# olga24912/lodestar

Hardware: AMD Instinct MI355X
Metric: verified signature sets/sec (node) (higher is better)
Workload: dtype u32/u64 (28-bit-limb Montgomery integer arithmetic); 1 GPU; C2 gossip attestation flood: 16384 single-pubkey sets per GPU, 1 set per batchable job; pk_mode=device table, sig_encoding=compressed 96 B, distinct_messages=16384, group_sets=1024, group_policy=0, inflight=32, slots=3, hw_queues=4, merge_sets=131072, pipeline_depth=3, parallelism=shard-by-job x1 (in-process devices), no collective

## Files before the change

lodestar_amd/csrc/helpers.cpp:

```cpp
#include "helper_layout.hpp"
#include "runtime_internal.hpp"

using namespace blsgpu_rt;
namespace hl = helper_layout;

static_assert(hl::kFp == W_FP && hl::kG1A == W_G1A && hl::kG1J == W_G1J && hl::kG2A == W_G2A && hl::kG2J == W_G2J &&
                  hl::kFp12 == W_FP12 && hl::kAwrTabWords == AWR_TAB_WORDS && hl::kMillerLineWords == kMillerLineWords,
              "helper_layout.hpp restates the element widths of kernels.h");

namespace {

template <class Body>
int helper_call(blsgpu_ctx* ctx, bool reads_table, Body body) {
  if (!enter(ctx)) return BLSGPU_ERR_CLOSED;
  struct Leave {
    blsgpu_ctx* ctx;
    ~Leave() { leave(ctx); }
  } leave_on_exit{ctx};
  Device& d = *ctx->devs[0];
  try {
    std::lock_guard<std::mutex> helper(d.helper_mu);
    std::shared_lock<std::shared_mutex> tl(d.table_mu, std::defer_lock);
    if (reads_table) tl.lock();
    HIPCHK(hipSetDevice(d.id));
// ... 447 lines not shown
    return BLSGPU_OK;
  });
}

int blsgpu_signing_roots(blsgpu_ctx* ctx, int kind, uint32_t n, const uint8_t* objects, uint32_t object_stride,
                         const uint8_t* domains, uint32_t domain_stride, uint8_t* out32) {
  if (!ctx || ctx->devs.empty() || !objects || !domains || !out32) return BLSGPU_ERR_ARGS;
  const uint32_t obj_len = kind == BLSGPU_ROOT_OBJECT ? 32 : (kind == BLSGPU_ROOT_ATTESTATION_DATA ? 128 : 0);
  if (!obj_len || object_stride < obj_len || (domain_stride != 0 && domain_stride < 32)) return BLSGPU_ERR_ARGS;
  if (n == 0) return BLSGPU_OK;
  return helper_call(ctx, false, [&](Device& d, Slot& sl, hipStream_t s) -> int {
    const hl::SigningRoots l(n, object_stride, domain_stride);
    sl.d_in.ensure(l.total);
    uint8_t* din = sl.d_in.p;
    HIPCHK(hipMemcpyAsync(din, objects, (size_t)n * object_stride, hipMemcpyHostToDevice, s));
    HIPCHK(hipMemcpyAsync(din + l.dom, domains, l.dom_bytes, hipMemcpyHostToDevice, s));
    launch_signing_roots(kind, din, n, object_stride, din + l.dom, domain_stride, din + l.out, s);
    HIPCHK(hipGetLastError());
    HIPCHK(hipMemcpyAsync(out32, din + l.out, 32 * (size_t)n, hipMemcpyDeviceToHost, s));
    HIPCHK(hipStreamSynchronize(s));
    return BLSGPU_OK;
  });
}

int blsgpu_debug_op(blsgpu_ctx* ctx, int op, uint32_t n, const uint8_t* in, uint32_t in_stride, uint8_t* out,
                    uint32_t out_stride, int32_t* status) {
  if (!ctx || ctx->devs.empty() || !in || !out || !status) return BLSGPU_ERR_ARGS;
  struct OpSize {
    int op;
    uint32_t in, out;
  };
  static const OpSize kOpSizes[] = {{0, 96, 48},    {1, 194, 192},  {2, 32, 192},   {3, 288, 576},  {4, 576, 576},
                                    {5, 104, 96},   {6, 200, 192},  {7, 64, 96},    {8, 32, 96},    {9, 200, 2880},
                                    {10, 104, 1440}, {11, 840, 56}, {16, 576, 576}, {17, 288, 576}, {18, 384, 192}};
  const OpSize* sz = nullptr;
  for (const OpSize& o : kOpSizes)
    if (o.op == op) sz = &o;
  if (!sz || in_stride < sz->in || out_stride < sz->out) return BLSGPU_ERR_ARGS;
  if (n == 0) return BLSGPU_OK;
  return helper_call(ctx, false, [&](Device& d, Slot& sl, hipStream_t s) -> int {
    struct Temp {
      void* p = nullptr;
      ~Temp() {
        if (p) (void)hipFree(p);
      }
    } din, dout, dst;
    HIPCHK(hipMalloc(&din.p, (size_t)n * in_stride));
    HIPCHK(hipMalloc(&dout.p, (size_t)n * out_stride));
    HIPCHK(hipMalloc(&dst.p, (size_t)n * 4));
    HIPCHK(hipMemcpyAsync(din.p, in, (size_t)n * in_stride, hipMemcpyHostToDevice, s));
    HIPCHK(hipMemsetAsync(dout.p, 0, (size_t)n * out_stride, s));
    launch_debug_op(op, n, (uint8_t*)din.p, in_stride, (uint8_t*)dout.p, out_stride, (int32_t*)dst.p, s);
    HIPCHK(hipGetLastError());
    HIPCHK(hipMemcpyAsync(out, dout.p, (size_t)n * out_stride, hipMemcpyDeviceToHost, s));
    HIPCHK(hipMemcpyAsync(status, dst.p, (size_t)n * 4, hipMemcpyDeviceToHost, s));
    HIPCHK(hipStreamSynchronize(s));
    return BLSGPU_OK;
  });
}

}
```

lodestar_amd/csrc/k_common.hpp:

```cpp
#pragma once
#include <atomic>

#include "kernels.h"
#include "ops.hpp"
#include "fp2x.hpp"

#define WAVE 64
#if defined(__HIP_DEVICE_COMPILE__) && !BLS_INLINE_PRODUCTS && !BLS_FP2_CLASSIC
static_assert(WAVE <= BLS_FP2_LDS_LANES, "fp2_mul LDS slot");
static_assert(2 * WAVE <= BLS_FP2_LDS_LANES, "128-lane kernels (gt_wave.hpp, k_msm_bucket) and fp2_mul LDS slot");
#endif

#ifndef BLSGPU_WPE
#define BLSGPU_WPE 1
#endif
#define STAGE_KERNEL __global__ __launch_bounds__(WAVE) __attribute__((amdgpu_waves_per_eu(BLSGPU_WPE, BLSGPU_WPE)))
#define STAGE_KERNEL_W(w) __global__ __launch_bounds__(WAVE) __attribute__((amdgpu_waves_per_eu(w, w)))
#ifndef BLSGPU_WPE_PK
#define BLSGPU_WPE_PK BLSGPU_WPE
#endif
#ifndef BLSGPU_WPE_HPREP
#define BLSGPU_WPE_HPREP 1
#endif
#ifndef BLSGPU_WPE_MSM
#define BLSGPU_WPE_MSM BLSGPU_WPE
#endif
#ifndef BLSGPU_WPE_LINES
#define BLSGPU_WPE_LINES BLSGPU_WPE
#endif
#ifndef BLSGPU_WPE_ACC
#define BLSGPU_WPE_ACC BLSGPU_WPE
#endif
#ifndef BLSGPU_WPE_DEC
#define BLSGPU_WPE_DEC BLSGPU_WPE
#endif
#ifndef BLSGPU_WPE_HASH
#define BLSGPU_WPE_HASH BLSGPU_WPE
#endif
#ifndef BLSGPU_WPE_HMAP
#define BLSGPU_WPE_HMAP 2
#endif
#ifndef BLSGPU_WPE_GRP
#define BLSGPU_WPE_GRP BLSGPU_WPE
#endif

__device__ __forceinline__ uint32_t opaque_u32(uint32_t x) {
  asm volatile("" : "+v"(x));
  return x;
}

__device__ __forceinline__ fp ld_fp(const uint32_t* p, uint32_t n, uint32_t i, int w0) {
  fp r;
// ... 154 lines not shown
  }
  return r;
}

template <class F>
__device__ jac<F> jac_mul_u64_j(const jac<F>& P, uint64_t k) {
  jac<F> r = jac_infinity<F>();
  if (k == 0) return r;
  int top = 63;
  while (((k >> top) & 1ull) == 0) top--;
  r = P;
  for (int i = top - 1; i >= 0; i--) {
    r = jac_dbl(r);
    if ((k >> i) & 1ull) r = jac_add(r, P);
  }
  return r;
}

template <class F>
__device__ __forceinline__ void tab_st(uint32_t* tab, uint32_t n, uint32_t i, int e, const jac<F>& v) {
  constexpr int WF = sizeof(F) / 4;
  const uint32_t* s = reinterpret_cast<const uint32_t*>(&v);
#pragma unroll
  for (int w = 0; w < 3 * WF; w++) tab[((size_t)e * 3 * WF + w) * n + i] = s[w];
}
template <class F>
__device__ __forceinline__ jac<F> tab_ld(const uint32_t* tab, uint32_t n, uint32_t i, int e) {
  constexpr int WF = sizeof(F) / 4;
  jac<F> v;
  uint32_t* d = reinterpret_cast<uint32_t*>(&v);
#pragma unroll
  for (int w = 0; w < 3 * WF; w++) d[w] = tab[((size_t)e * 3 * WF + w) * n + i];
  return v;
}
BLS_HD int scalar_word_digit(uint64_t w, int k, bool& neg) {
  const int d = 2 * (int)((w >> (4 * k)) & 15u) - 15;
  neg = d < 0;
  return (d < 0 ? -d : d) >> 1;
}
template <class F>
__device__ jac<F> jac_mul_scalar_word(const jac<F>& P, uint64_t w, uint32_t* tab, uint32_t n, uint32_t i) {
  const jac<F> P2 = jac_dbl(P);
  jac<F> t = P;
  tab_st(tab, n, i, 0, t);
#pragma unroll 1
  for (int e = 1; e < 8; e++) {
    t = jac_add(t, P2);
    tab_st(tab, n, i, e, t);
  }
  const uint32_t ii = opaque_u32(i);
  auto term = [&](int k, bool hi) {
    bool neg;
    const int e = scalar_word_digit(w, hi ? k + 8 : k, neg);
    jac<F> q = tab_ld<F>(tab, n, ii, e);
    if (hi) q = endo_lambda(q);
    return neg ? jac_neg(q) : q;
  };
  jac<F> r = jac_add(term(7, false), term(7, true));
#pragma unroll 1
  for (int k = 6; k >= 0; k--) {
    r = jac_dbl(jac_dbl(jac_dbl(jac_dbl(r))));
    r = jac_add(r, term(k, false));
    r = jac_add(r, term(k, true));
  }
  return r;
}

template <class F>
__device__ jac<F> jac_mul_words(const jac<F>& P, const uint32_t* k, int nw) {
  jac<F> r = jac_infinity<F>();
  for (int i = 32 * nw - 1; i >= 0; i--) {
// ... 34 lines not shown
```

lodestar_amd/csrc/k_debug.hip:

```cpp
#include "k_common.hpp"
#include "gt_wave.hpp"

__device__ fp dbg_load_fp(const uint8_t* b) {
  fp x;
  fp_from_be48_plain(b, x, 0xff);
  return fp_to_mont(x);
}
__device__ fp2 dbg_load_fp2(const uint8_t* b) { return fp2_make(dbg_load_fp(b + 48), dbg_load_fp(b)); }
__device__ g2a dbg_load_g2(const uint8_t* b) {
  g2a p;
  p.x = dbg_load_fp2(b);
  p.y = dbg_load_fp2(b + 96);
  return p;
}
__device__ g1a dbg_load_g1(const uint8_t* b) {
  g1a p;
  p.x = dbg_load_fp(b);
  p.y = dbg_load_fp(b + 48);
  return p;
}
__device__ void dbg_store_fp12(const fp12& f, uint8_t* b) {
  const fp2* c[6] = {&f.c0.c0, &f.c0.c1, &f.c0.c2, &f.c1.c0, &f.c1.c1, &f.c1.c2};
  for (int k = 0; k < 6; k++) {
    fp_to_be48(c[k]->c0, b + 96 * k);
// ... 82 lines not shown
      g1a pk;
      st = jac_to_aff(jac_mul_words(jac_from_aff(g), w, 8), pk) ? 0 : -1;
      if (st == 0) g1a_to_be96(pk, o);
      break;
    }
    case 9: {
      uint64_t w = 0;
      for (int j = 0; j < 8; j++) w |= (uint64_t)a[192 + j] << (8 * j);
      g2a r;
      uint32_t* tab = reinterpret_cast<uint32_t*>(o + 192);
      st = jac_to_aff(jac_mul_scalar_word(jac_from_aff(dbg_load_g2(a)), w, tab, 1, 0), r) ? 0 : -1;
      if (st == 0) g2a_to_be192(r, o);
      break;
    }
    case 10: {
      uint64_t w = 0;
      for (int j = 0; j < 8; j++) w |= (uint64_t)a[96 + j] << (8 * j);
      g1a r;
      uint32_t* tab = reinterpret_cast<uint32_t*>(o + 96);
      st = jac_to_aff(jac_mul_scalar_word(jac_from_aff(dbg_load_g1(a)), w, tab, 1, 0), r) ? 0 : -1;
      if (st == 0) g1a_to_be96(r, o);
      break;
    }
    case 11: {
      const uint32_t* w = reinterpret_cast<const uint32_t*>(a);
      fp x[15];
      for (int k = 0; k < 15; k++)
        for (int j = 0; j < BLS_NL; j++) x[k].l[j] = w[14 * k + j];
      const fp r = fp_lc(T<1>(x[0]), T<1>(x[1]), T<1>(x[2]), T<1>(x[3]), T<1>(x[4]), T<1>(x[5]), T<1>(x[6]),
                         T<-1>(x[7]), T<-1>(x[8]), T<-1>(x[9]), T<-1>(x[10]), T<-1>(x[11]), T<-1>(x[12]), T<-1>(x[13]),
                         T<-1>(x[14]));
      uint32_t* ow = reinterpret_cast<uint32_t*>(o);
      for (int j = 0; j < BLS_NL; j++) ow[j] = r.l[j];
      break;
    }
    default:
      st = -2;
  }
  status[i] = st;
}

__global__ __launch_bounds__(GTW_MILLER_LANES) void k_debug_gt(int op, const uint8_t* in, uint32_t in_stride, uint8_t* out,
                                                         uint32_t out_stride, int32_t* status) {
  __shared__ GtwLds sh;
  const uint32_t i = blockIdx.x, t = threadIdx.x;
  const uint8_t* a = in + (size_t)i * in_stride;
  uint8_t* o = out + (size_t)i * out_stride;
  if (op == 16) {
    if (t == 0) gtw_from_reg(sh.F, dbg_load_fp12(a));
    gtw_sync();
    gtw_final_exp(sh.F, sh.W, sh.S, t);
  } else {
    if (t == 0) {
      const g1a P = dbg_load_g1(a);
      const g2a Q = dbg_load_g2(a + 96);
      lds_st(sh.QA, 0, Q.x.c0);
      lds_st(sh.QA, 1, Q.x.c1);
      lds_st(sh.QA, 2, Q.y.c0);
      lds_st(sh.QA, 3, Q.y.c1);
      lds_st(sh.L, 0, P.x);
      lds_st(sh.L, 1, P.y);
    }
    gtw_sync();
    const fp xP = lds_ld(sh.L, 0), yP = lds_ld(sh.L, 1);
    gtw_sync();
    gtw_miller_loop(sh.F, sh.QA, xP, yP, sh.TB, sh.L, sh.L1, sh.S, sh.S2, t);
// ... 87 lines not shown
```

lodestar_amd/csrc/k_pk.hip:

```cpp
#include "k_common.hpp"

#ifndef BLSGPU_PK_AGG_GROUPS
#define BLSGPU_PK_AGG_GROUPS 1
#endif
__global__ __launch_bounds__(WAVE) void k_pk_aggregate(PipelineBuffers b, uint32_t n_sets) {
  __shared__ uint32_t red[WAVE * W_G1J];
  __shared__ uint32_t err_k[WAVE];
  __shared__ int32_t err_c[WAVE];
  if (blockIdx.x >= n_sets) return;
  const uint32_t set = b.agg_sets ? b.agg_sets[blockIdx.x] : blockIdx.x;
  uint32_t lane = threadIdx.x;
  int8_t* agg_status = b.status + 2 * b.n;
  const uint32_t first = b.set_pk_first[set], last = b.set_pk_first[set + 1];
  g1j acc = jac_infinity<fp>();
  uint32_t my_err_k = 0xffffffffu;
  int my_err = 0;
  for (uint32_t k = first + lane; k < last; k += WAVE) {
    g1a q;
    if (b.pk_bytes) {
      uint8_t raw[96];
      const uint8_t* src = b.pk_bytes + (size_t)k * 96;
#pragma unroll
      for (int t = 0; t < 96; t++) raw[t] = src[t];
      bool inf = false;
// ... 146 lines not shown
      uint4 v = src[k];
      uint32_t w[4] = {v.x, v.y, v.z, v.w};
#pragma unroll
      for (int j = 0; j < 16; j++) raw[16 * k + j] = (uint8_t)(w[j >> 2] >> (8 * (j & 3)));
    }
    g1a a;
    bool inf = false;
    int st = pk_decode96(raw, a, inf);
    if (st == BLS_OK && inf) st = BLS_PK_IS_INFINITY;
    if (st == BLS_OK) P = jac_from_aff(a);
    return st;
  }
  if (b.set_pk_first[i + 1] == b.set_pk_first[i]) return BLS_EMPTY_AGGREGATE;
  const int st = b.status[2 * b.n + i];
  if (st) return st;
  P = ld_g1j(b.pk_jac, b.n, i);
  return jac_is_inf(P) ? BLS_PK_IS_INFINITY : BLS_OK;
}

STAGE_KERNEL_W(BLSGPU_WPE_PK) void k_pk_finish(PipelineBuffers b, uint32_t n_sets, int8_t* pk_status) {
  uint32_t i = blockIdx.x * WAVE + threadIdx.x;
  if (i >= n_sets) return;
  g1j P;
  int st = set_pubkey(b, i, P);
  g1j R = jac_infinity<fp>();
  if (st == BLS_OK) {
    const uint64_t w = b.scalars[i];
    R = (w == 0) ? P : jac_mul_scalar_word(P, w, b.scal_tab, b.n, i);
  }
  st_g1j(b.pk_jac, b.n, i, R);
  pk_status[i] = (int8_t)st;
}

STAGE_KERNEL void k_unit_aggregate(PipelineBuffers b) {
  uint32_t u = blockIdx.x * WAVE + threadIdx.x;
  if (u >= b.n_units) return;
  const uint32_t a = b.unit_set_first[u], e = b.unit_set_first[u + 1];
  g1a out;
  out.x = fp_zero();
  out.y = fp_zero();
  bool ok = false;
  if (e - a == 1) {
    const uint32_t i = b.unit_sets[a];
    if (b.include[i]) {
      out = ld_g1a(b.pk_aff, b.n, i);
      ok = true;
    }
  } else {
    g1j acc = jac_infinity<fp>();
    for (uint32_t k = a; k < e; k++) {
      const uint32_t i = b.unit_sets[k];
      if (b.include[i]) acc = jac_add_aff(acc, ld_g1a(b.pk_aff, b.n, i));
    }
    ok = jac_to_aff(acc, out);
  }
  st_g1a(b.unit_p, b.n, u, out);
  b.unit_ok[u] = ok ? 1 : 0;
}

__global__ __launch_bounds__(WAVE) void k_pk_serialize(PipelineBuffers b, uint32_t n_sets, uint8_t* out,
                                                       uint32_t out_len) {
  uint32_t i = blockIdx.x * WAVE + threadIdx.x;
  if (i >= n_sets) return;
  int st = b.set_pk_first[i + 1] == b.set_pk_first[i] ? BLS_EMPTY_AGGREGATE : b.status[2 * b.n + i];
  uint8_t buf[96];
  for (int k = 0; k < 96; k++) buf[k] = 0;
// ... 21 lines not shown
  for (uint32_t k = 0; k < 96; k++) raw[k] = k < pk_len ? src[k] : 0;
  g1a a;
  const int st = pk_key_validate(raw, pk_len, a);
  uint8_t buf[96];
  for (int k = 0; k < 96; k++) buf[k] = 0;
  if (st == BLS_OK) g1a_to_be96(a, buf);
  if (out96)
    for (int k = 0; k < 96; k++) out96[(size_t)i * 96 + k] = buf[k];
  status[i] = (int8_t)st;
}

__global__ __launch_bounds__(WAVE) void k_pk_table_fill(const uint8_t* pk96, uint32_t n, uint32_t* table_dst,
                                                        int8_t* status) {
  uint32_t i = blockIdx.x * WAVE + threadIdx.x;
  if (i >= n) return;
  uint8_t raw[96];
  for (int k = 0; k < 96; k++) raw[k] = pk96[(size_t)i * 96 + k];
  g1a a;
  bool inf = false;
  int st = pk_decode96(raw, a, inf);
  if (st == BLS_OK && inf) st = BLS_PK_IS_INFINITY;
  uint32_t* dst = table_dst + (size_t)i * W_PKTAB;
  for (int l = 0; l < BLS_NL; l++) {
    dst[l] = st == BLS_OK ? a.x.l[l] : 0;
    dst[BLS_NL + l] = st == BLS_OK ? a.y.l[l] : 0;
  }
  dst[2 * BLS_NL] = 0;
  dst[2 * BLS_NL + 1] = 0;
  dst[2 * BLS_NL + 2] = 0;
  dst[2 * BLS_NL + 3] = 0;
  status[i] = (int8_t)st;
}

static inline dim3 grid_for(uint32_t n) { return dim3((n + WAVE - 1) / WAVE); }

void launch_pk_aggregate(const PipelineBuffers& b, uint32_t n, hipStream_t s) {
  if (b.agg_sets) n = b.n_agg;
  if (!n) return;
  const uint32_t lanes = 1024 * WAVE;
  if ((uint64_t)n * 64 <= lanes || !BLSGPU_PK_AGG_GROUPS)
    hipLaunchKernelGGL(k_pk_aggregate, dim3(n), dim3(WAVE), 0, s, b, n);
  else if ((uint64_t)n * 32 <= 2 * lanes)
    hipLaunchKernelGGL(k_pk_aggregate_g<32>, dim3((n * 32 + WAVE - 1) / WAVE), dim3(WAVE), 0, s, b, n);
  else if ((uint64_t)n * 16 <= 2 * lanes)
    hipLaunchKernelGGL(k_pk_aggregate_g<16>, dim3((n * 16 + WAVE - 1) / WAVE), dim3(WAVE), 0, s, b, n);
  else
    hipLaunchKernelGGL(k_pk_aggregate_g<8>, dim3((n * 8 + WAVE - 1) / WAVE), dim3(WAVE), 0, s, b, n);
}
void launch_pk_finish(const PipelineBuffers& b, uint32_t n, hipStream_t s) {
  if (n) hipLaunchKernelGGL(k_pk_finish, grid_for(n), dim3(WAVE), 0, s, b, n, b.status + b.n);
}
void launch_unit_aggregate(const PipelineBuffers& b, hipStream_t s) {
  if (b.n_units) hipLaunchKernelGGL(k_unit_aggregate, grid_for(b.n_units), dim3(WAVE), 0, s, b);
}
void launch_pk_serialize(const PipelineBuffers& b, uint32_t n, uint8_t* out, uint32_t out_len, hipStream_t s) {
  if (n) hipLaunchKernelGGL(k_pk_serialize, grid_for(n), dim3(WAVE), 0, s, b, n, out, out_len);
}
void launch_key_validate(const uint8_t* pks, uint32_t n, uint32_t pk_len, uint32_t stride, uint8_t* out96,
                         int8_t* status, hipStream_t s) {
  if (n) hipLaunchKernelGGL(k_key_validate, grid_for(n), dim3(WAVE), 0, s, pks, n, pk_len, stride, out96, status);
}
void launch_pk_table_fill(const uint8_t* pk96, uint32_t n, uint32_t* table_dst, int8_t* status, hipStream_t s) {
  if (n) hipLaunchKernelGGL(k_pk_table_fill, grid_for(n), dim3(WAVE), 0, s, pk96, n, table_dst, status);
}
```

lodestar_amd/csrc/kernels.h:

```cpp
#pragma once
#include <hip/hip_runtime.h>
#include <stdint.h>
#include <vector>

#define W_FP 14
#define W_G1A (2 * W_FP)
#define W_G1J (3 * W_FP)
#define W_G2A (4 * W_FP)
#define W_G2J (6 * W_FP)
#define W_FP12 (12 * W_FP)
#define W_PKTAB 32
#define MILLER_STEPS 68
#define W_LINE (3 * 2 * W_FP)

#define SF_SIG_INF 1u
#define MF_H_INF 1u

struct PipelineBuffers {
  uint32_t n;
  const uint8_t* sigs;
  const uint32_t* sig_len;
  uint32_t sig_stride;
  const uint8_t* pk_bytes;
  const uint32_t* set_pk_first;
  const uint32_t* pk_index;
  const uint32_t* pk_table;
  uint32_t pk_table_n;
  const uint32_t* agg_sets;
  uint32_t n_agg;
  uint32_t pk_direct1;
  const uint64_t* scalars;
  uint32_t* scal_tab;
  const uint32_t* job_first_set;
  uint32_t n_jobs;
  const uint8_t* umsgs;
  const uint32_t* msg_idx;
  uint32_t n_umsg;
  uint32_t nm;
  uint32_t n_units;
  const uint32_t* unit_set_first;
  const uint32_t* unit_sets;
  const uint32_t* unit_msg;
  uint32_t* sig_aff;
  uint32_t* h_aff;
  uint32_t* h_jac;
  uint32_t* h_norm;
  uint32_t* h_prep;
  uint32_t* h_q;
  uint32_t* inv_buf;
  uint32_t* inv_buf_pk;
  uint32_t* pk_jac;
  uint32_t* pk_aff;
  uint32_t* rsig;
  uint32_t* unit_p;
  uint32_t n_chunks;
  const uint32_t* chunk_first;
  const uint32_t* chunk_items;
  uint32_t* f_chunk;
  uint32_t* lines;
  uint8_t* flags;
// ... 37 lines not shown
  uint32_t dbl[MILLER_MAX_SEGS];
};
void launch_miller_acc(const PipelineBuffers& b, bool units, hipStream_t s, const MillerSegs* segs = nullptr);
void launch_miller_acc2(const PipelineBuffers& b, bool units, hipStream_t s);
void launch_miller_acc6(const PipelineBuffers& b, bool units, hipStream_t s);
#ifndef BLSGPU_EXCLUSIVE_SMALL
#define BLSGPU_EXCLUSIVE_SMALL 1
#endif
void launch_miller_coop(const PipelineBuffers& b, bool units, hipStream_t s, bool exclusive = false);
void launch_group_reduce(const PipelineBuffers& b, const uint32_t* f_ranges, uint32_t n_groups, uint32_t* F,
                         hipStream_t s);
void launch_group_tree(const PipelineBuffers& b, const uint32_t* f_ranges, uint32_t n_groups, const uint32_t* runs,
                       uint32_t n_runs, const uint32_t* pairs, const std::vector<uint32_t>& level_end, uint32_t* F,
                       hipStream_t s, const MillerSegs* segs = nullptr, uint32_t* H = nullptr);
void launch_group_check(const uint32_t* S, const uint32_t* F, uint32_t n_groups, uint8_t* ok, hipStream_t s,
                        const uint32_t* sel = nullptr, uint32_t n_sel = 0, const uint32_t* G = nullptr,
                        bool exclusive = false, bool lane = false);
void launch_group_check6(const uint32_t* F, const uint32_t* G, uint32_t n_groups, uint8_t* ok, hipStream_t s,
                         const uint32_t* sel = nullptr, uint32_t n_sel = 0);
void launch_check6_miller(const uint32_t* S, const uint32_t* F, uint32_t n_groups, uint8_t* ok, hipStream_t s,
                          const uint32_t* sel, uint32_t n_sel, uint32_t* lines, uint8_t* flags);
void launch_group_sig_miller_sel(const uint32_t* S, uint32_t n_groups, const uint32_t* sel, uint32_t n_sel, uint32_t* G,
                                 hipStream_t s);
void launch_group_sig_miller(const uint32_t* S, uint32_t n_groups, uint32_t* G, hipStream_t s, bool exclusive = false,
                             bool lane = false);
void launch_copy_words(uint32_t* dst, const uint32_t* src, size_t n, hipStream_t s);
void launch_group_reduce_lane(const PipelineBuffers& b, const uint32_t* set_ranges, const uint32_t* f_ranges,
                              uint32_t n_groups, uint32_t* S, uint32_t* F, hipStream_t s);
void launch_range_combine_lane(const uint32_t* S_in, const uint32_t* F_in, uint32_t n_in, const uint32_t* ranges,
                               uint32_t n_out, uint32_t* S_out, uint32_t* F_out, hipStream_t s);
void launch_range_combine(const uint32_t* S_in, const uint32_t* F_in, uint32_t n_in, const uint32_t* ranges,
                          uint32_t n_out, uint32_t* S_out, uint32_t* F_out, hipStream_t s);
void launch_pk_table_fill(const uint8_t* pk96, uint32_t n, uint32_t* table_dst, int8_t* status, hipStream_t s);
void launch_pk_serialize(const PipelineBuffers& b, uint32_t n_sets, uint8_t* out, uint32_t out_len, hipStream_t s);
void launch_key_validate(const uint8_t* pks, uint32_t n, uint32_t pk_len, uint32_t stride, uint8_t* out96,
                         int8_t* status, hipStream_t s);
inline uint32_t sig_agg_lanes(uint32_t n_groups, uint32_t n_sigs) {
  if (n_groups == 0) return 1;
  const uint64_t n = n_groups, lanes = 1024 * 64;
  const uint32_t by_count = n * 64 <= lanes ? 64 : n * 32 <= 2 * lanes ? 32 : n * 16 <= 2 * lanes ? 16
                            : n * 8 <= 2 * lanes ? 8 : 1;
  const uint64_t mean = ((uint64_t)n_sigs + n - 1) / n;
  const uint32_t by_size = mean <= 3 ? 1 : mean <= 8 ? 8 : mean <= 16 ? 16 : mean <= 32 ? 32 : 64;
  return by_count < by_size ? by_count : by_size;
}
void launch_sig_aggregate(const PipelineBuffers& b, const uint32_t* group_first, uint32_t n_groups, uint32_t n_sigs,
                          uint32_t* agg, int8_t* agg_status, uint32_t* first_bad, hipStream_t s);
void launch_sig_agg_serialize(const uint32_t* group_first, uint32_t n_groups, const uint32_t* agg, int8_t* agg_status,
                              uint8_t* out, uint32_t out_len, hipStream_t s);
struct AwrBuffers {
  uint32_t n;
  uint32_t n_groups;
  const uint32_t* group_first;
  const uint64_t* words;
  const uint8_t* pk_bytes;
  const uint32_t* pk_index;
  const uint32_t* pk_table;
  uint32_t pk_table_n;
  const uint32_t* sig_aff;
  const uint8_t* sig_flags;
  const int8_t* sig_status;
  uint32_t* tab;
  uint32_t tab_n;
  uint32_t* sum_pk;
  uint32_t* sum_sig;
  uint32_t* err_k;
// ... 31 lines not shown
```

lodestar_amd/csrc/runtime.cpp:

```cpp
#include <pthread.h>
#include <stdio.h>
#include <sys/random.h>

#include <cmath>
#include <string>
#include <system_error>

#include "runtime_internal.hpp"
#include "miller_plan.hpp"

using namespace blsgpu_rt;

namespace {

std::atomic<int64_t> g_fail_run_skip{0}, g_fail_run_count{0};
thread_local bool tl_dispatcher = false;

inline uint32_t chunk_size(uint32_t len, uint32_t min_per_chunk) {
  const uint32_t count = min_per_chunk ? len / min_per_chunk : 0;
  return count <= 1 ? len : (len + count - 1) / count;
}

struct GroupPlanEntry {
  uint32_t first, end;
// ... 461 lines not shown
  const size_t ob_flags = 0, ob_mflags = al256(n), ob_unit = al256(ob_mflags + nm), ob_status = al256(ob_unit + n),
               ob_include = al256(ob_status + 3 * (size_t)stride), ob_spec = al256(ob_include + stride),
               bytes_total = al256(ob_spec + stride);
  sl.d_bytes.ensure(bytes_total);
  const uint32_t max_ranges = std::max<uint32_t>(std::max(ng0, nj), 1);
  const size_t o_ok = al256(nj), res_bytes = o_ok + max_ranges;
  sl.d_res.ensure(res_bytes);
  sl.h_res.ensure(res_bytes);
  sl.d_S.ensure((size_t)W_G2J * max_ranges);
  sl.d_F.ensure((size_t)W_FP12 * max_ranges);
  sl.d_G.ensure((size_t)W_FP12 * std::max<uint32_t>(ng0, 1));
  sl.d_msmB.ensure((size_t)MSM_BUCKET_WORDS * std::max<uint32_t>(n_slices, 1));
  sl.d_msmW.ensure((size_t)MSM_WINDOW_WORDS * max_ranges);
  const size_t per_set = W_G2A + W_G1J + W_G1A + W_FP12 + 8 * W_G1J + 2 * W_FP + (merged ? W_G1A : 0);
  sl.d_work.ensure((size_t)stride * per_set + (size_t)nm * (W_G2A + W_G2J + W_FP + 14 * W_FP + 2 * W_G2J));
  sl.d_lines.ensure((size_t)nm * kMillerLineWords);
  if (keep_f) sl.d_fkeep.ensure((size_t)stride * W_FP12);
  if (segs > 1) sl.d_fseg.ensure((size_t)W_FP12 * n_franges);
  if (rsig_spec) sl.d_fb.ensure((size_t)stride * 9 * W_G2J);
  uint8_t* const din = sl.d_in.p;
  uint8_t* const d_ok0 = sl.d_res.p + o_ok;

  PipelineBuffers pb;
  memset(&pb, 0, sizeof pb);
  pb.n = stride;
  pb.sigs = din + o_sigs;
  pb.sig_len = reinterpret_cast<uint32_t*>(din + o_siglen);
  pb.sig_stride = sig_w;
  pb.pk_bytes = table_mode ? nullptr : din + (bytes_agg ? o_pk2 : o_pk);
  pb.set_pk_first = (table_mode || bytes_agg) ? reinterpret_cast<uint32_t*>(din + o_pk) : nullptr;
  pb.pk_index = table_mode ? reinterpret_cast<uint32_t*>(din + o_pk2) : nullptr;
  pb.pk_table = d.table.p;
  pb.pk_table_n = d.table_n;
  pb.agg_sets = reinterpret_cast<uint32_t*>(din + o_agg);
  pb.n_agg = (uint32_t)agg_sets.size();
  pb.pk_direct1 = 1;
  pb.scalars = reinterpret_cast<uint64_t*>(din + o_scal);
  pb.job_first_set = reinterpret_cast<uint32_t*>(din + o_jobs);
  pb.n_jobs = nj;
  pb.umsgs = din + o_umsg;
  pb.msg_idx = reinterpret_cast<uint32_t*>(din + o_midx);
  pb.n_umsg = n_umsg;
  pb.nm = nm;
  pb.n_units = n_units;
  pb.unit_set_first = reinterpret_cast<uint32_t*>(din + o_ufirst);
  pb.unit_sets = reinterpret_cast<uint32_t*>(din + o_usets);
  pb.unit_msg = reinterpret_cast<uint32_t*>(din + o_umsgi);
  uint32_t* w = sl.d_work.p;
  pb.sig_aff = w; w += (size_t)stride * W_G2A;
  pb.pk_jac = w; w += (size_t)stride * W_G1J;
  pb.pk_aff = w; w += (size_t)stride * W_G1A;
  pb.rsig = nullptr;
  pb.f_chunk = w; w += (size_t)stride * W_FP12;
  pb.scal_tab = w; w += (size_t)stride * 8 * W_G1J;
  if (merged) {
    pb.unit_p = w; w += (size_t)stride * W_G1A;
  }
  pb.n_chunks = n_chunks;
  pb.chunk_first = reinterpret_cast<uint32_t*>(din + o_cfirst);
  pb.chunk_items = reinterpret_cast<uint32_t*>(din + o_citems);
  pb.inv_buf = w; w += (size_t)stride * W_FP;
  pb.inv_buf_pk = w; w += (size_t)stride * W_FP;
  pb.h_aff = w; w += (size_t)nm * W_G2A;
  pb.h_jac = w; w += (size_t)nm * W_G2J;
  pb.h_norm = w; w += (size_t)nm * W_FP;
  pb.h_prep = w; w += (size_t)nm * 14 * W_FP;
// ... 1084 lines not shown
  }
  d->q_cv.notify_all();
  for (size_t k = 0; k < joins.size(); k++) {
    try {
      joins[k].join();
      free_slot(d, gone[k]);
    } catch (std::system_error&) {
      joins[k].detach();
    }
  }
}

void destroy_device(Device* d) {
  {
    std::lock_guard<std::mutex> lk(d->q_mu);
    d->stop = true;
  }
  d->q_cv.notify_all();
  for (auto& t : d->workers) t.join();
  if (d->uworker.joinable()) d->uworker.join();
  for (Slot* s : d->slots) free_slot(d, s);
  if (d->uslot) free_slot(d, d->uslot);
  (void)hipSetDevice(d->id);
  for (hipStream_t st : d->st)
    if (st) (void)hipStreamSynchronize(st), (void)hipStreamDestroy(st);
  for (hipStream_t st : d->ust)
    if (st) (void)hipStreamSynchronize(st), (void)hipStreamDestroy(st);
  for (hipStream_t st : d->same_st)
    if (st) (void)hipStreamSynchronize(st), (void)hipStreamDestroy(st);
  for (hipEvent_t e : d->same_ev)
    if (e) (void)hipEventDestroy(e);
  d->helper.release_all();
  d->table.release();
  if (d->table_stream) (void)hipStreamDestroy(d->table_stream);
  delete d;
}

int64_t hw_queues_of_process() {
  const char* v = getenv("GPU_MAX_HW_QUEUES");
  const long q = v ? strtol(v, nullptr, 10) : 0;
  return q > 0 ? q : 4;
}

int64_t default_slots(int64_t) { return 3; }

int ensure_slots(blsgpu_ctx* ctx) {
  std::lock_guard<std::mutex> lk(ctx->slots_mu);
  if (ctx->slots_started) return BLSGPU_OK;
  try {
    for (Device* d : ctx->devs) {
      if (!d->st[0]) {
        d->blocking_sync = ctx->blocking_sync != 0;
        create_streams(ctx, d);
      }
      resize_slots(d, ctx->slots_per_device);
      if (!d->uslot) {
        Slot* u = new Slot();
        u->urgent = true;
        try {
          u->set_stream(d->ust[0]);
          create_slot_events(d, u);
        } catch (HipError&) {
          free_slot(d, u);
          throw;
        }
        d->uslot = u;
// ... 106 lines not shown
    for (uint32_t j = 0; j < b->n_jobs; j++) job_result[j] = (int8_t)-code;
}

Options snapshot(blsgpu_ctx* ctx) {
  std::lock_guard<std::mutex> lk(ctx->opt_mu);
  return ctx->opt;
}

}

extern "C" {

int blsgpu_init(const int* devices, int n_devices, blsgpu_ctx** out) {
  if (!out) return BLSGPU_ERR_ARGS;
  *out = nullptr;
  int count = 0;
  if (hipGetDeviceCount(&count) != hipSuccess || count <= 0) return BLSGPU_ERR_NO_DEVICE;
  std::vector<int> ids;
  if (devices && n_devices > 0) {
    for (int i = 0; i < n_devices; i++) {
      if (devices[i] < 0 || devices[i] >= count) return BLSGPU_ERR_ARGS;
      ids.push_back(devices[i]);
    }
  } else {
    for (int i = 0; i < count; i++) ids.push_back(i);
  }
  blsgpu_ctx* ctx = new blsgpu_ctx();
  ctx->hw_queues = hw_queues_of_process();
  ctx->slots_per_device = default_slots(ctx->hw_queues);
  if (const char* v = getenv("BLSGPU_MILLER_SEGMENTS")) {
    const long j = strtol(v, nullptr, 10);
    if (j >= 1 && j <= MILLER_MAX_SEGS) ctx->opt.miller_segments = j;
  }
  try {
    for (int id : ids) {
      Device* d = new Device();
      d->id = id;
      ctx->devs.push_back(d);
      HIPCHK(hipSetDevice(id));
      HIPCHK(hipStreamCreateWithFlags(&d->table_stream, hipStreamNonBlocking));
    }
  } catch (HipError&) {
    blsgpu_destroy(ctx);
    return BLSGPU_ERR_NO_DEVICE;
  }
  *out = ctx;
  return BLSGPU_OK;
}

void blsgpu_destroy(blsgpu_ctx* ctx) {
  if (!ctx) return;
  {
    std::unique_lock<std::mutex> lk(ctx->active_mu);
    ctx->closed = true;
    ctx->active_cv.wait(lk, [&] { return ctx->active == 0; });
  }
  for (Device* d : ctx->devs) destroy_device(d);
  delete ctx;
}

int blsgpu_device_count(const blsgpu_ctx* ctx) { return ctx ? (int)ctx->devs.size() : 0; }

uint32_t blsgpu_pubkeys_count(const blsgpu_ctx* ctx) {
  if (!ctx || ctx->devs.empty()) return 0;
  uint32_t n = UINT32_MAX;
  for (Device* d : ctx->devs) {
    std::shared_lock<std::shared_mutex> lk(d->table_mu);
    n = std::min(n, d->table_n);
  }
  return n;
}

int blsgpu_pubkeys_upload(blsgpu_ctx* ctx, uint32_t first_index, const uint8_t* pk96, uint32_t n) {
  if (!ctx) return BLSGPU_ERR_ARGS;
  if (n == 0) return BLSGPU_OK;
  if (!pk96) return BLSGPU_ERR_ARGS;
  if (!enter(ctx)) return BLSGPU_ERR_CLOSED;
  std::lock_guard<std::mutex> tl(ctx->table_mu);
  int result = BLSGPU_OK;
  for (Device* d : ctx->devs) {
    std::shared_lock<std::shared_mutex> lk(d->table_mu);
    if (first_index > d->table_n) result = BLSGPU_ERR_ARGS;
  }
  auto upload_one = [&](Device* d) -> int {
    try {
      HIPCHK(hipSetDevice(d->id));
      hipStream_t ts = d->table_stream;
      const uint32_t need = first_index + n;
      uint8_t* dpk = nullptr;
      int8_t* dst = nullptr;
      uint32_t* tmp = nullptr;
      HIPCHK(hipMalloc((void**)&dpk, (size_t)n * 96));
      HIPCHK(hipMalloc((void**)&dst, n));
      HIPCHK(hipMalloc((void**)&tmp, (size_t)n * W_PKTAB * 4));
      HIPCHK(hipMemcpyAsync(dpk, pk96, (size_t)n * 96, hipMemcpyHostToDevice, ts));
      launch_pk_table_fill(dpk, n, tmp, dst, ts);
      HIPCHK(hipGetLastError());
      std::vector<int8_t> hst(n);
      HIPCHK(hipMemcpyAsync(hst.data(), dst, n, hipMemcpyDeviceToHost, ts));
      HIPCHK(hipStreamSynchronize(ts));
      int err = 0;
      for (uint32_t i = 0; i < n && !err; i++) err = hst[i];
      if (!err) {
        std::unique_lock<std::shared_mutex> lk(d->table_mu);
        if (need > d->table.cap / W_PKTAB) {
          DevBuf<uint32_t> nt;
          nt.ensure((size_t)std::max<uint32_t>(need, d->table_n + d->table_n / 2) * W_PKTAB);
          if (d->table_n)
            HIPCHK(hipMemcpyAsync(nt.p, d->table.p, (size_t)d->table_n * W_PKTAB * 4, hipMemcpyDeviceToDevice, ts));
          d->table.release();
          d->table = nt;
        }
        HIPCHK(hipMemcpyAsync(d->table.p + (size_t)first_index * W_PKTAB, tmp, (size_t)n * W_PKTAB * 4,
                              hipMemcpyDeviceToDevice, ts));
        HIPCHK(hipStreamSynchronize(ts));
        d->table_n = std::max(d->table_n, need);
      }
      (void)hipFree(dpk);
      (void)hipFree(dst);
      (void)hipFree(tmp);
      return err;
    } catch (HipError&) {
      return BLSGPU_DEVICE_ERROR;
    } catch (std::exception&) {
      return BLSGPU_DEVICE_ERROR;
    }
  };
  if (!result) {
    std::vector<int> rc(ctx->devs.size(), 0);
    if (ctx->devs.size() == 1) {
      rc[0] = upload_one(ctx->devs[0]);
    } else {
      std::vector<std::thread> th;
      for (size_t k = 0; k < ctx->devs.size(); k++) th.emplace_back([&, k] { rc[k] = upload_one(ctx->devs[k]); });
      for (auto& t : th) t.join();
    }
    for (int r : rc)
      if (r && !result) result = r;
  }
  leave(ctx);
  return result;
}

int blsgpu_set_option(blsgpu_ctx* ctx, const char* key, int64_t value) {
  if (!ctx || !key) return BLSGPU_ERR_ARGS;
  std::string k(key);
  if (k == "urgent_cus" || k == "urgent_isolate" || k == "blocking_sync" || k == "pipeline_prio") {
    std::lock_guard<std::mutex> sk(ctx->slots_mu);
    if (ctx->slots_started) return BLSGPU_ERR_ARGS;
    if (k == "blocking_sync" || k == "pipeline_prio") {
      if (value < 0 || value > 1) return BLSGPU_ERR_ARGS;
      (k == "blocking_sync" ? ctx->blocking_sync : ctx->pipeline_prio) = value;
    } else if (k == "urgent_cus") {
// ... 413 lines not shown
```

lodestar_amd/csrc/runtime_internal.hpp:

```cpp
#pragma once
#include <hip/hip_runtime.h>
#include <stdint.h>
#include <stdlib.h>
#include <string.h>

#include <algorithm>
#include <atomic>
#include <chrono>
#include <condition_variable>
#include <deque>
#include <mutex>
#include <shared_mutex>
#include <thread>
#include <vector>

#include "../../include/blsgpu.h"
#include "batch_rand.hpp"
#include "kernels.h"

namespace blsgpu_rt __attribute__((visibility("hidden"))) {

struct HipError {
  hipError_t e;
};
// ... 141 lines not shown
    d_msmB.release(); d_msmW.release(); d_fb.release(); d_G.release(); d_fkeep.release(); d_fseg.release();
    h_in.release(); h_res.release(); h_ok.release(); h_list.release();
  }
};

struct Call;
struct Task {
  Call* call;
  uint32_t shard;
};

enum { kSig = 0, kMsg = 1, kPk = 2, kTail = 3, kStreams = 4, kMaxPairs = 3 };
#ifndef BLSGPU_STREAM_PRIO
#define BLSGPU_STREAM_PRIO ((1 << kMsg) | (1 << kTail))
#endif
#ifndef BLSGPU_STREAM_PAIRS
#define BLSGPU_STREAM_PAIRS 1
#endif


struct Device {
  int id = 0;
  hipStream_t table_stream = nullptr;
  hipStream_t st[2 * kMaxPairs] = {};
  int npairs = 2;
  std::mutex enq_mu;
  std::mutex helper_mu;
  Slot helper;
  hipStream_t same_st[2] = {};
  hipEvent_t same_ev[3] = {};
  std::shared_mutex table_mu;
  DevBuf<uint32_t> table;
  uint32_t table_n = 0;
  std::mutex q_mu;
  std::condition_variable q_cv;
  std::deque<Task> queue;
  bool stop = false;
  std::vector<Slot*> slots;
  std::vector<std::thread> workers;
  int runs_inflight = 0;
  std::atomic<uint32_t> run_seq{0};
  std::atomic<int64_t> load{0};
  hipStream_t ust[4] = {};
  std::vector<uint32_t> umask;
  int uprio = 0;
  std::deque<Task> uqueue;
  Slot* uslot = nullptr;
  std::thread uworker;
  std::atomic<int> upending{0};
  std::atomic<uint64_t> spurious_groups{0};
  int urgent_cus = 0;
  std::vector<uint32_t> main_mask;
  bool blocking_sync = true;
  std::mutex fail_mu;
  double fail_rate = 0;
};

struct Options {
  int64_t group_sets = 1024;
  int64_t max_devices = 64;
  bool profile = false;
  bool dedupe = true;
  int64_t miller_k = 0;
  int64_t merge_sets = 131072;
  int64_t merge_wait_us = 2000;
  int64_t idle_wait_us = 0;
// ... 130 lines not shown
```

Measured before the change: 4.248 million sets/s.

## Precompute per-pubkey affine multiple tables for table-mode scalar multiplication

At pubkey table upload, each key gets a 16-entry table of affine odd multiples (P and 2^16·P bases) built with one batched inversion and stored in a new device buffer. In table mode with single-key sets, the pk-finish stage then runs a fixed-window scalar multiply that loads these precomputed affine points and uses mixed additions plus the GLV endomorphism. This replaces building a per-set Jacobian table of multiples for every verification. The cost is 16x more device memory per key and extra upload-time work. A fallback path disables the table when any key fails to build.

Result: slower. 4.200 million sets/s (-1.1%).

```diff
diff --git a/lodestar_amd/csrc/helpers.cpp b/lodestar_amd/csrc/helpers.cpp
--- a/lodestar_amd/csrc/helpers.cpp
+++ b/lodestar_amd/csrc/helpers.cpp
@@ -503,11 +503,13 @@
   };
   static const OpSize kOpSizes[] = {{0, 96, 48},    {1, 194, 192},  {2, 32, 192},   {3, 288, 576},  {4, 576, 576},
                                     {5, 104, 96},   {6, 200, 192},  {7, 64, 96},    {8, 32, 96},    {9, 200, 2880},
-                                    {10, 104, 1440}, {11, 840, 56}, {16, 576, 576}, {17, 288, 576}, {18, 384, 192}};
+                                    {10, 104, 1440}, {11, 840, 56}, {12, 104, 96 + W_PKMULT * 4},
+                                    {16, 576, 576}, {17, 288, 576}, {18, 384, 192}};
   const OpSize* sz = nullptr;
   for (const OpSize& o : kOpSizes)
     if (o.op == op) sz = &o;
   if (!sz || in_stride < sz->in || out_stride < sz->out) return BLSGPU_ERR_ARGS;
+  if (op == 12 && out_stride % 4) return BLSGPU_ERR_ARGS;
   if (n == 0) return BLSGPU_OK;
   return helper_call(ctx, false, [&](Device& d, Slot& sl, hipStream_t s) -> int {
     struct Temp {
diff --git a/lodestar_amd/csrc/k_common.hpp b/lodestar_amd/csrc/k_common.hpp
--- a/lodestar_amd/csrc/k_common.hpp
+++ b/lodestar_amd/csrc/k_common.hpp
@@ -4,6 +4,7 @@
 #include "kernels.h"
 #include "ops.hpp"
 #include "fp2x.hpp"
+#include "pk_mult.hpp"
 
 #define WAVE 64
 #if defined(__HIP_DEVICE_COMPILE__) && !BLS_INLINE_PRODUCTS && !BLS_FP2_CLASSIC
@@ -18,6 +19,9 @@
 #define STAGE_KERNEL_W(w) __global__ __launch_bounds__(WAVE) __attribute__((amdgpu_waves_per_eu(w, w)))
 #ifndef BLSGPU_WPE_PK
 #define BLSGPU_WPE_PK BLSGPU_WPE
+#endif
+#ifndef BLSGPU_WPE_PKTAB
+#define BLSGPU_WPE_PKTAB 2
 #endif
 #ifndef BLSGPU_WPE_HPREP
 #define BLSGPU_WPE_HPREP 1
@@ -238,11 +242,6 @@
 #pragma unroll
   for (int w = 0; w < 3 * WF; w++) d[w] = tab[((size_t)e * 3 * WF + w) * n + i];
   return v;
-}
-BLS_HD int scalar_word_digit(uint64_t w, int k, bool& neg) {
-  const int d = 2 * (int)((w >> (4 * k)) & 15u) - 15;
-  neg = d < 0;
-  return (d < 0 ? -d : d) >> 1;
 }
 template <class F>
 __device__ jac<F> jac_mul_scalar_word(const jac<F>& P, uint64_t w, uint32_t* tab, uint32_t n, uint32_t i) {
diff --git a/lodestar_amd/csrc/k_debug.hip b/lodestar_amd/csrc/k_debug.hip
--- a/lodestar_amd/csrc/k_debug.hip
+++ b/lodestar_amd/csrc/k_debug.hip
@@ -138,6 +138,19 @@
                          T<-1>(x[14]));
       uint32_t* ow = reinterpret_cast<uint32_t*>(o);
       for (int j = 0; j < BLS_NL; j++) ow[j] = r.l[j];
+      break;
+    }
+    case 12: {
+      uint64_t w = 0;
+      for (int j = 0; j < 8; j++) w |= (uint64_t)a[96 + j] << (8 * j);
+      uint32_t* rec = reinterpret_cast<uint32_t*>(o + 96);
+      g1a r;
+      if (!pk_mult_build(dbg_load_g1(a), rec)) {
+        st = -1;
+        break;
+      }
+      st = jac_to_aff(g1_mul_word_tab([&](int k) { return pk_mult_entry(rec, k); }, w), r) ? 0 : -1;
+      if (st == 0) g1a_to_be96(r, o);
       break;
     }
     default:
diff --git a/lodestar_amd/csrc/k_pk.hip b/lodestar_amd/csrc/k_pk.hip
--- a/lodestar_amd/csrc/k_pk.hip
+++ b/lodestar_amd/csrc/k_pk.hip
@@ -202,6 +202,52 @@
   pk_status[i] = (int8_t)st;
 }
 
+__device__ __forceinline__ g1a ld_pkmult(const uint32_t* mult, uint32_t idx, int k) {
+  const uint4* q = reinterpret_cast<const uint4*>(mult + (size_t)idx * PKM_KEY_WORDS + (size_t)k * PKM_ENTRY_WORDS);
+  uint32_t w[2 * BLS_NL];
+#pragma unroll
+  for (int t = 0; t < 2 * BLS_NL / 4; t++) {
+    const uint4 v = q[t];
+    w[4 * t] = v.x;
+    w[4 * t + 1] = v.y;
+    w[4 * t + 2] = v.z;
+    w[4 * t + 3] = v.w;
+  }
+  g1a r;
+#pragma unroll
+  for (int l = 0; l < BLS_NL; l++) {
+    r.x.l[l] = w[l];
+    r.y.l[l] = w[BLS_NL + l];
+  }
+  return r;
+}
+
+STAGE_KERNEL_W(BLSGPU_WPE_PKTAB) void k_pk_finish_tab(PipelineBuffers b, uint32_t n_sets, int8_t* pk_status) {
+  uint32_t i = blockIdx.x * WAVE + threadIdx.x;
+  if (i >= n_sets) return;
+  const uint32_t first = b.set_pk_first[i], cnt = b.set_pk_first[i + 1] - first;
+  g1j R = jac_infinity<fp>();
+  int st = BLS_OK;
+  if (cnt == 0) {
+    st = BLS_EMPTY_AGGREGATE;
+  } else {
+    const uint32_t idx = b.pk_index[first];
+    if (cnt != 1 || idx >= b.pk_table_n) {
+      st = BLS_DEVICE_ERROR;
+    } else {
+      const uint64_t w = b.scalars[i];
+      if (w == 0) {
+        R = jac_from_aff(ld_pktab(b.pk_table, idx));
+      } else {
+        const uint32_t* mult = b.pk_mult;
+        R = g1_mul_word_tab([&](int k) { return ld_pkmult(mult, idx, k); }, w);
+      }
+    }
+  }
+  st_g1j(b.pk_jac, b.n, i, R);
+  pk_status[i] = (int8_t)st;
+}
+
 STAGE_KERNEL void k_unit_aggregate(PipelineBuffers b) {
   uint32_t u = blockIdx.x * WAVE + threadIdx.x;
   if (u >= b.n_units) return;
@@ -289,6 +335,20 @@
   status[i] = (int8_t)st;
 }
 
+static_assert(PKM_ENTRY_WORDS == W_PKTAB && PKM_KEY_WORDS == W_PKMULT, "a multiple is stored as a table row");
+__global__ __launch_bounds__(WAVE) void k_pk_mult_fill(const uint32_t* rows, const int8_t* status, uint32_t n,
+                                                       uint32_t* mult_dst, uint8_t* ok) {
+  uint32_t i = blockIdx.x * WAVE + threadIdx.x;
+  if (i >= n) return;
+  uint32_t* o = mult_dst + (size_t)i * PKM_KEY_WORDS;
+  if (status[i] != BLS_OK) {
+    for (int l = 0; l < PKM_KEY_WORDS; l++) o[l] = 0;
+    ok[i] = 0;
+    return;
+  }
+  ok[i] = pk_mult_build(ld_pktab(rows, i), o) ? 1 : 0;
+}
+
 static inline dim3 grid_for(uint32_t n) { return dim3((n + WAVE - 1) / WAVE); }
 
 void launch_pk_aggregate(const PipelineBuffers& b, uint32_t n, hipStream_t s) {
@@ -305,7 +365,11 @@
     hipLaunchKernelGGL(k_pk_aggregate_g<8>, dim3((n * 8 + WAVE - 1) / WAVE), dim3(WAVE), 0, s, b, n);
 }
 void launch_pk_finish(const PipelineBuffers& b, uint32_t n, hipStream_t s) {
-  if (n) hipLaunchKernelGGL(k_pk_finish, grid_for(n), dim3(WAVE), 0, s, b, n, b.status + b.n);
+  if (!n) return;
+  if (b.pk_mult && !b.pk_bytes && b.set_pk_first && b.pk_index && b.pk_direct1 && b.n_agg == 0)
+    hipLaunchKernelGGL(k_pk_finish_tab, grid_for(n), dim3(WAVE), 0, s, b, n, b.status + b.n);
+  else
+    hipLaunchKernelGGL(k_pk_finish, grid_for(n), dim3(WAVE), 0, s, b, n, b.status + b.n);
 }
 void launch_unit_aggregate(const PipelineBuffers& b, hipStream_t s) {
   if (b.n_units) hipLaunchKernelGGL(k_unit_aggregate, grid_for(b.n_units), dim3(WAVE), 0, s, b);
@@ -320,3 +384,7 @@
 void launch_pk_table_fill(const uint8_t* pk96, uint32_t n, uint32_t* table_dst, int8_t* status, hipStream_t s) {
   if (n) hipLaunchKernelGGL(k_pk_table_fill, grid_for(n), dim3(WAVE), 0, s, pk96, n, table_dst, status);
 }
+void launch_pk_mult_fill(const uint32_t* rows, const int8_t* status, uint32_t n, uint32_t* mult_dst, uint8_t* ok,
+                         hipStream_t s) {
+  if (n) hipLaunchKernelGGL(k_pk_mult_fill, grid_for(n), dim3(WAVE), 0, s, rows, status, n, mult_dst, ok);
+}
diff --git a/lodestar_amd/csrc/kernels.h b/lodestar_amd/csrc/kernels.h
--- a/lodestar_amd/csrc/kernels.h
+++ b/lodestar_amd/csrc/kernels.h
@@ -26,6 +26,7 @@
   const uint32_t* pk_index;
   const uint32_t* pk_table;
   uint32_t pk_table_n;
+  const uint32_t* pk_mult;
   const uint32_t* agg_sets;
   uint32_t n_agg;
   uint32_t pk_direct1;
@@ -129,6 +130,9 @@
 void launch_range_combine(const uint32_t* S_in, const uint32_t* F_in, uint32_t n_in, const uint32_t* ranges,
                           uint32_t n_out, uint32_t* S_out, uint32_t* F_out, hipStream_t s);
 void launch_pk_table_fill(const uint8_t* pk96, uint32_t n, uint32_t* table_dst, int8_t* status, hipStream_t s);
+#define W_PKMULT (16 * W_PKTAB)
+void launch_pk_mult_fill(const uint32_t* rows, const int8_t* status, uint32_t n, uint32_t* mult_dst, uint8_t* ok,
+                         hipStream_t s);
 void launch_pk_serialize(const PipelineBuffers& b, uint32_t n_sets, uint8_t* out, uint32_t out_len, hipStream_t s);
 void launch_key_validate(const uint8_t* pks, uint32_t n, uint32_t pk_len, uint32_t stride, uint8_t* out96,
                          int8_t* status, hipStream_t s);
diff --git a/lodestar_amd/csrc/pk_mult.hpp b/lodestar_amd/csrc/pk_mult.hpp
--- /dev/null
+++ b/lodestar_amd/csrc/pk_mult.hpp
@@ -0,0 +1,97 @@
+#pragma once
+#include "curve.hpp"
+
+#define PKM_ENTRY_WORDS 32
+#define PKM_ENTRIES 16
+#define PKM_KEY_WORDS (PKM_ENTRIES * PKM_ENTRY_WORDS)
+#define PKM_FLAG_WORD 28
+
+BLS_HD int scalar_word_digit(uint64_t w, int k, bool& neg) {
+  const int d = 2 * (int)((w >> (4 * k)) & 15u) - 15;
+  neg = d < 0;
+  return (d < 0 ? -d : d) >> 1;
+}
+
+BLS_HDNI bool pk_mult_build(const g1a& P, uint32_t* out) {
+  fp z[PKM_ENTRIES], pre[PKM_ENTRIES];
+  bool ok = true;
+  g1j base = jac_from_aff(P);
+#pragma unroll 1
+  for (int h = 0; h < 2; h++) {
+    if (h == 1) {
+#pragma unroll 1
+      for (int i = 0; i < 16; i++) base = jac_dbl(base);
+    }
+    const g1j two = jac_dbl(base);
+    g1j t = base;
+#pragma unroll 1
+    for (int e = 0; e < 8; e++) {
+      if (e) t = jac_add(t, two);
+      const int k = 8 * h + e;
+      uint32_t* o = out + k * PKM_ENTRY_WORDS;
+      for (int l = 0; l < BLS_NL; l++) {
+        o[l] = t.x.l[l];
+        o[BLS_NL + l] = t.y.l[l];
+      }
+      for (int l = 2 * BLS_NL; l < PKM_ENTRY_WORDS; l++) o[l] = 0;
+      ok = ok && !jac_is_inf(t);
+      z[k] = t.z;
+      pre[k] = k ? fp_mul(pre[k - 1], t.z) : t.z;
+    }
+  }
+  if (!ok) {
+    for (int l = 0; l < PKM_KEY_WORDS; l++) out[l] = 0;
+    return false;
+  }
+  fp inv = fp_inv(pre[PKM_ENTRIES - 1]);
+#pragma unroll 1
+  for (int k = PKM_ENTRIES - 1; k >= 0; k--) {
+    const fp zi = k ? fp_mul(inv, pre[k - 1]) : inv;
+    if (k) inv = fp_mul(inv, z[k]);
+    const fp zi2 = fp_sqr(zi);
+    uint32_t* o = out + k * PKM_ENTRY_WORDS;
+    fp x, y;
+    for (int l = 0; l < BLS_NL; l++) {
+      x.l[l] = o[l];
+      y.l[l] = o[BLS_NL + l];
+    }
+    x = fp_mul(x, zi2);
+    y = fp_mul(y, fp_mul(zi2, zi));
+    for (int l = 0; l < BLS_NL; l++) {
+      o[l] = x.l[l];
+      o[BLS_NL + l] = y.l[l];
+    }
+  }
+  out[PKM_FLAG_WORD] = 1;
+  return true;
+}
+
+BLS_HD g1a pk_mult_entry(const uint32_t* rec, int k) {
+  g1a q;
+  for (int l = 0; l < BLS_NL; l++) {
+    q.x.l[l] = rec[k * PKM_ENTRY_WORDS + l];
+    q.y.l[l] = rec[k * PKM_ENTRY_WORDS + BLS_NL + l];
+  }
+  return q;
+}
+
+template <class LoadEntry>
+BLS_INL g1j g1_mul_word_tab(LoadEntry entry, uint64_t w) {
+  g1j r = jac_infinity<fp>();
+#pragma unroll 1
+  for (int j = 3; j >= 0; j--) {
+    if (j != 3) r = jac_dbl(jac_dbl(jac_dbl(jac_dbl(r))));
+#pragma unroll 1
+    for (int t = 0; t < 4; t++) {
+      const int h = t >> 1;
+      const bool hi = t & 1;
+      bool neg;
+      const int e = scalar_word_digit(w, (hi ? 8 : 0) + 4 * h + j, neg);
+      g1a q = entry(8 * h + e);
+      if (hi) q.x = fp_mul(q.x, G1_BETA);
+      q.y = fp_select(neg, fp_neg(q.y), q.y);
+      r = jac_add_aff(r, q);
+    }
+  }
+  return r;
+}
diff --git a/lodestar_amd/csrc/runtime.cpp b/lodestar_amd/csrc/runtime.cpp
--- a/lodestar_amd/csrc/runtime.cpp
+++ b/lodestar_amd/csrc/runtime.cpp
@@ -517,6 +517,7 @@
   pb.pk_index = table_mode ? reinterpret_cast<uint32_t*>(din + o_pk2) : nullptr;
   pb.pk_table = d.table.p;
   pb.pk_table_n = d.table_n;
+  pb.pk_mult = (table_mode && d.mult_on && !d.mult_off) ? d.mult.p : nullptr;
   pb.agg_sets = reinterpret_cast<uint32_t*>(din + o_agg);
   pb.n_agg = (uint32_t)agg_sets.size();
   pb.pk_direct1 = 1;
@@ -1667,6 +1668,7 @@
     if (e) (void)hipEventDestroy(e);
   d->helper.release_all();
   d->table.release();
+  d->mult.release();
   if (d->table_stream) (void)hipStreamDestroy(d->table_stream);
   delete d;
 }
@@ -1839,10 +1841,13 @@
     const long j = strtol(v, nullptr, 10);
     if (j >= 1 && j <= MILLER_MAX_SEGS) ctx->opt.miller_segments = j;
   }
+  bool pk_mult = true;
+  if (const char* v = getenv("BLSGPU_PK_MULT")) pk_mult = !(v[0] == '0' && v[1] == 0);
   try {
     for (int id : ids) {
       Device* d = new Device();
       d->id = id;
+      d->mult_on = pk_mult;
       ctx->devs.push_back(d);
       HIPCHK(hipSetDevice(id));
       HIPCHK(hipStreamCreateWithFlags(&d->table_stream, hipStreamNonBlocking));
@@ -1897,6 +1902,13 @@
       uint8_t* dpk = nullptr;
       int8_t* dst = nullptr;
       uint32_t* tmp = nullptr;
+      uint32_t* mtmp = nullptr;
+      uint8_t* mok = nullptr;
+      bool with_mult;
+      {
+        std::shared_lock<std::shared_mutex> lk(d->table_mu);
+        with_mult = d->mult_on && !d->mult_off;
+      }
       HIPCHK(hipMalloc((void**)&dpk, (size_t)n * 96));
       HIPCHK(hipMalloc((void**)&dst, n));
       HIPCHK(hipMalloc((void**)&tmp, (size_t)n * W_PKTAB * 4));
@@ -1904,12 +1916,36 @@
       launch_pk_table_fill(dpk, n, tmp, dst, ts);
       HIPCHK(hipGetLastError());
       std::vector<int8_t> hst(n);
+      std::vector<uint8_t> hok;
       HIPCHK(hipMemcpyAsync(hst.data(), dst, n, hipMemcpyDeviceToHost, ts));
+      if (with_mult) {
+        HIPCHK(hipMalloc((void**)&mtmp, (size_t)n * W_PKMULT * 4));
+        HIPCHK(hipMalloc((void**)&mok, n));
+        launch_pk_mult_fill(tmp, dst, n, mtmp, mok, ts);
+        HIPCHK(hipGetLastError());
+        hok.resize(n);
+        HIPCHK(hipMemcpyAsync(hok.data(), mok, n, hipMemcpyDeviceToHost, ts));
+      }
       HIPCHK(hipStreamSynchronize(ts));
       int err = 0;
       for (uint32_t i = 0; i < n && !err; i++) err = hst[i];
       if (!err) {
         std::unique_lock<std::shared_mutex> lk(d->table_mu);
+        for (uint32_t i = 0; i < n && with_mult; i++)
+          if (!hok[i]) d->mult_off = true, with_mult = false;
+        if (with_mult) {
+          if (need > d->mult.cap / W_PKMULT) {
+            DevBuf<uint32_t> nm;
+            nm.ensure((size_t)std::max<uint32_t>(need, d->table_n + d->table_n / 2) * W_PKMULT);
+            if (d->table_n)
+              HIPCHK(hipMemcpyAsync(nm.p, d->mult.p, (size_t)d->table_n * W_PKMULT * 4, hipMemcpyDeviceToDevice, ts));
+            HIPCHK(hipStreamSynchronize(ts));
+            d->mult.release();
+            d->mult = nm;
+          }
+          HIPCHK(hipMemcpyAsync(d->mult.p + (size_t)first_index * W_PKMULT, mtmp, (size_t)n * W_PKMULT * 4,
+                                hipMemcpyDeviceToDevice, ts));
+        }
         if (need > d->table.cap / W_PKTAB) {
           DevBuf<uint32_t> nt;
           nt.ensure((size_t)std::max<uint32_t>(need, d->table_n + d->table_n / 2) * W_PKTAB);
@@ -1926,6 +1962,8 @@
       (void)hipFree(dpk);
       (void)hipFree(dst);
       (void)hipFree(tmp);
+      if (mtmp) (void)hipFree(mtmp);
+      if (mok) (void)hipFree(mok);
       return err;
     } catch (HipError&) {
       return BLSGPU_DEVICE_ERROR;
diff --git a/lodestar_amd/csrc/runtime_internal.hpp b/lodestar_amd/csrc/runtime_internal.hpp
--- a/lodestar_amd/csrc/runtime_internal.hpp
+++ b/lodestar_amd/csrc/runtime_internal.hpp
@@ -197,6 +197,9 @@
   std::shared_mutex table_mu;
   DevBuf<uint32_t> table;
   uint32_t table_n = 0;
+  DevBuf<uint32_t> mult;
+  bool mult_on = true;
+  bool mult_off = false;
   std::mutex q_mu;
   std::condition_variable q_cv;
   std::deque<Task> queue;
```
